# miemie2013/Pytorch-PPYOLO

Measured on AMD Instinct MI355X. Metric: images/sec PPYOLO R50-vd 608x608 bs=8, higher is better.
Workload: dtype f32; 1 GPU; PPYOLO ResNet50-vd (DCNv2, CoordConv, SPP) 608x608, 8 images per GPU, device-resident input -> padded detections; global_batch=8, parallelism=single GPU, hip_graph=True, tile_table=tuned_gfx950_f16x2.json

## Files before the change

pytorch-ppyolo_amd/ppyolo_hip/csrc/conv_shared.h:

```cpp
#pragma once
#include "common.h"

#ifndef PPY_X3_BBLOCK
#define PPY_X3_BBLOCK 1
#endif

struct ConvArgs {
    const float *x, *w, *scale, *shift, *res, *posb;
    const unsigned short *w3;
    const unsigned short *wf16;
    const float *scale_f16;
    const float *posb_f16;
    const float *amax_in;
    const float *amax_in2 = nullptr;
    float *amax_out;
    float *y, *part;
    int x_ld, res_ld, y_ld;
    int N, H, W, C, Ho, Wo, K, R, S, stride, pad, act, ups;
    int M, Kred, cchunks, chunks_total, chunks_per_split;
    int nstages;
    int panel_n = 0;
    unsigned long long *trace;
    float *bn_part = nullptr;
    int *bn_slices_host = nullptr;
    int bn_capacity = 0;
    int bn_nostore = 0;
    const float *bn_mean = nullptr, *bn_invstd = nullptr, *bn_gamma = nullptr, *bn_beta = nullptr;
    float *yscale = nullptr;
    float ysplit_mul = 0.f, ysplit_add = 0.f;
    const float *xscale = nullptr;
};

static __device__ __forceinline__ float split_scale_of(float bound) {
    const int e = (int)((__float_as_uint(bound) >> 23) & 0xffu);
    int f = 267 - e;
    f = f < 103 ? 103 : (f > 167 ? 167 : f);
    return __uint_as_float((unsigned)f << 23);
}
static __device__ __forceinline__ float pow2_above(float mx) {
    const unsigned e = (__float_as_uint(mx) >> 23) & 0xffu;
    return __uint_as_float((e >= 253u ? 254u : e + 1u) << 23);
}
static __device__ __forceinline__ float pow2_inverse(float s) {
    return __uint_as_float((254u - ((__float_as_uint(s) >> 23) & 0xffu)) << 23);
}

#if defined(__HIPCC__)
static __device__ __forceinline__ float conv_amax_in(const ConvArgs &p, int n) {
    float mx = amax_read(p.amax_in, n);
    if (p.amax_in2) mx = fmaxf(mx, amax_read(p.amax_in2, n));
    return mx;
}
#endif

struct Geometry {
    int Ho, Wo, M, Kred, chunks;
};

static inline ppy_conv_cfg_info ppy_cfg_info(int family, int local, int operands, int bm, int bn, int stages, int splitk_mode,
                                             bool reads_presplit, bool writes_presplit, bool bn_stats, int stats_twin = -1) {
    return ppy_conv_cfg_info{family, local, operands, bm, bn, stages, splitk_mode, reads_presplit, writes_presplit, bn_stats, stats_twin};
}

int ppy_x3_num_configs();
int ppy_x3_f16_base();
int ppy_x3_config_info(int local_cfg, ppy_conv_cfg_info *out);
int ppy_x3_dispatch(const ConvArgs &p, int local_cfg, int splits, hipStream_t stream);
static inline int ppy_panel_n(const ConvArgs &p, int BM, int BN, int splits) {
    static const int mode = getenv("PPY_TILE_PANEL") ? atoi(getenv("PPY_TILE_PANEL")) : 1;
    if (mode == 0 || splits > 1) return 0;
    const int tiles_m = (p.M + BM - 1) / BM, tiles_n = (p.K + BN - 1) / BN;
    if (tiles_m * tiles_n < 16) return 0;
    const double A = (double)p.N * p.H * p.W * p.C * 4.0, W = (double)p.K * p.Kred * 4.0;
    int best = 1;
    double best_cost = A + 8.0 * W;
    for (int gn = 2; gn <= 8; gn *= 2) {
        if (gn > tiles_n || 8 / gn > tiles_m) continue;
        if (mode > 1 && gn != mode) continue;
        const double cost = gn * A + (8.0 / gn) * W;
        if (cost < 0.9 * best_cost || (mode > 1 && gn == mode)) { best = gn; best_cost = cost; }
    }
    return best == 1 ? 0 : (tiles_n + best - 1) / best;
}
#if defined(__HIPCC__)
__device__ __forceinline__ void ppy_tile_of(const ConvArgs &p, int tiles_n, int &tile_m, int &tile_n) {
    const int nb = (int)gridDim.x, q = nb >> 3, r = nb & 7;
    const int xcd = (int)blockIdx.x & 7, idx = (int)blockIdx.x >> 3;
    const int tile_id = xcd * q + min(xcd, r) + idx;
    const int pn = p.panel_n;
    if (pn <= 0 || pn >= tiles_n) {
        tile_m = tile_id / tiles_n;
        tile_n = tile_id - tile_m * tiles_n;
        return;
    }
    const int tiles_m = nb / tiles_n, per_panel = tiles_m * pn;
    const int panel = tile_id / per_panel, within = tile_id - panel * per_panel;
    const int pw = min(pn, tiles_n - panel * pn);
    tile_m = within / pw;
    tile_n = panel * pn + (within - tile_m * pw);
}
#endif

int ppy_stream_num_configs();
int ppy_stream_config_info(int local_cfg, ppy_conv_cfg_info *out);
int ppy_stream_dispatch(const ConvArgs &p, int local_cfg, float *pool, int pool_ld, hipStream_t stream);
int ppy_patch_num_configs();
int ppy_patch_config_info(int local_cfg, ppy_conv_cfg_info *out);
int ppy_patch_dispatch(const ConvArgs &p, int local_cfg, hipStream_t stream);
int ppy_patch_maxpool_dispatch(const ConvArgs &p, int Hp, int Wp, hipStream_t stream);
int ppy_ws_num_configs();
int ppy_ws_config_info(int local_cfg, ppy_conv_cfg_info *out);
int ppy_ws_dispatch(const ConvArgs &p, int local_cfg, int splits, hipStream_t stream);
int ppy_small_num_configs();
int ppy_small_config_info(int local_cfg, ppy_conv_cfg_info *out);
int ppy_small_dispatch(const ConvArgs &p, int local_cfg, int splits, hipStream_t stream);

namespace {

constexpr int BK = 32;
constexpr int LDS_LD = 36;

typedef __attribute__((ext_vector_type(8))) __bf16 bf16x8;
typedef __attribute__((ext_vector_type(2))) __bf16 bf16x2;
typedef __attribute__((ext_vector_type(2))) float floatx2;
typedef __attribute__((ext_vector_type(4))) unsigned uintx4;
typedef __attribute__((ext_vector_type(8))) _Float16 f16x8;
typedef __attribute__((ext_vector_type(2))) _Float16 f16x2;

__device__ __forceinline__ unsigned cvt_pk_f16(float a, float b) {
    const floatx2 v = {a, b};
    return __builtin_bit_cast(unsigned, __builtin_convertvector(v, f16x2));
}
__device__ __forceinline__ float f16_lo(unsigned p) { return (float)__builtin_bit_cast(_Float16, (unsigned short)(p & 0xffffu)); }
__device__ __forceinline__ float f16_hi(unsigned p) { return (float)__builtin_bit_cast(_Float16, (unsigned short)(p >> 16)); }

__device__ __forceinline__ unsigned cvt_pk_bf16(float a, float b) {
    const floatx2 v = {a, b};
    return __builtin_bit_cast(unsigned, __builtin_convertvector(v, bf16x2));
}

__device__ __forceinline__ float epilogue_store(const ConvArgs &p, int m, int col, float v,
                                                float sc, float sh) {
    const int hw = p.Ho * p.Wo;
    if (p.posb) v += p.posb[(long long)(m % hw) * p.K + col];
    v = fmaf(v, sc, sh);
    if (p.res) v += p.res[(long long)m * p.res_ld + col];
    v = ppy_apply_act(v, p.act);
    if (!p.ups) {
        p.y[(long long)m * p.y_ld + col] = v;
    } else {
        const int n = m / hw, rem = m - n * hw;
        const int ho = rem / p.Wo, wo = rem - ho * p.Wo;
        const long long W2 = 2LL * p.Wo;
        float *o = p.y + (((long long)n * 2 * p.Ho + 2 * ho) * W2 + 2 * wo) * p.y_ld + col;
        o[0] = v;
        o[p.y_ld] = v;
        o[W2 * p.y_ld] = v;
        o[(W2 + 1) * p.y_ld] = v;
    }
    return v;
}

template <int TM, int TN, int WM, int WN, bool SPLIT, bool VEC>
__device__ __forceinline__ void tile_epilogue(const ConvArgs &p, floatx16 (&acc)[TM][TN], float *smem, int m0,
                                              int n0, int wm, int wn, int lane, int wave, int split,
                                              const float (*rowscale)[4] = nullptr, const float (*rowsplit)[4] = nullptr,
                                              bool split_out = false) {
    const int hw = p.Ho * p.Wo;
    if constexpr (VEC) {
        float *sE = smem + wave * (32 * LDS_LD);
        const int erow = lane >> 3, ec4 = (lane & 7) * 4;
        const int mw0 = min(m0 + wm * WM, p.M - 1), mw1 = min(m0 + wm * WM + WM - 1, p.M - 1);
        const int n_lo = mw0 / hw, n_hi = mw1 / hw;
        const int bnd = (n_lo + 1) * hw;
        float amx = 0.0f, amx_hi = 0.0f;
        floatx4 rv[TM][TN][4];
        if (!SPLIT && p.res) {
#pragma unroll
            for (int j = 0; j < TN; ++j)
#pragma unroll
                for (int i = 0; i < TM; ++i)
#pragma unroll
                    for (int t = 0; t < 4; ++t) {
                        const int col = n0 + wn * WN + j * 32 + ec4;
                        const int m = m0 + wm * WM + i * 32 + erow + 8 * t;
                        rv[i][j][t] = floatx4{0.f, 0.f, 0.f, 0.f};
                        if (col < p.K && m < p.M)
                            rv[i][j][t] = *reinterpret_cast<const floatx4 *>(p.res + (long long)m * p.res_ld + col);
                    }
        } else if (!SPLIT && p.posb) {
#pragma unroll
            for (int j = 0; j < TN; ++j)
#pragma unroll
                for (int i = 0; i < TM; ++i)
#pragma unroll
                    for (int t = 0; t < 4; ++t) {
                        const int col = n0 + wn * WN + j * 32 + ec4;
                        const int m = m0 + wm * WM + i * 32 + erow + 8 * t;
                        rv[i][j][t] = floatx4{0.f, 0.f, 0.f, 0.f};
                        if (col < p.K && m < p.M)
                            rv[i][j][t] = *reinterpret_cast<const floatx4 *>(p.posb + (long long)(m % hw) * p.K + col);
                    }
        }
        constexpr bool HOIST_SC = TM * TN < 4;
        floatx4 scv[HOIST_SC ? TN : 1], shv[HOIST_SC ? TN : 1];
        if constexpr (HOIST_SC) {
#pragma unroll
            for (int j = 0; j < TN; ++j) {
                const int col = n0 + wn * WN + j * 32 + ec4;
                scv[j] = floatx4{1.f, 1.f, 1.f, 1.f};
                shv[j] = floatx4{0.f, 0.f, 0.f, 0.f};
                if (!SPLIT && col < p.K) {
                    scv[j] = *reinterpret_cast<const floatx4 *>(p.scale + col);
                    shv[j] = *reinterpret_cast<const floatx4 *>(p.shift + col);
                }
            }
            if (!SPLIT) {
#pragma unroll
                for (int j = 0; j < TN; ++j) asm volatile("" : "+v"(scv[j]), "+v"(shv[j]));
            }
        }
        if (!SPLIT && (p.res || p.posb)) {
#pragma unroll
            for (int j = 0; j < TN; ++j)
#pragma unroll
                for (int i = 0; i < TM; ++i)
#pragma unroll
                    for (int t = 0; t < 4; ++t) asm volatile("" : "+v"(rv[i][j][t]));
        }
#pragma unroll
        for (int j = 0; j < TN; ++j) {
            const int col = n0 + wn * WN + j * 32 + ec4;
            const bool colok = col < p.K;
            floatx4 sc = {1.f, 1.f, 1.f, 1.f}, sh = {0.f, 0.f, 0.f, 0.f};
            if constexpr (HOIST_SC) {
                sc = scv[j];
                sh = shv[j];
            } else if (!SPLIT) {
                if (colok) {
                    sc = *reinterpret_cast<const floatx4 *>(p.scale + col);
                    sh = *reinterpret_cast<const floatx4 *>(p.shift + col);
                }
                asm volatile("" : "+v"(sc), "+v"(sh));
            }
#pragma unroll
            for (int i = 0; i < TM; ++i) {
                const int mbase = m0 + wm * WM + i * 32 + erow;
#pragma unroll
                for (int e = 0; e < 16; ++e) {
                    const int row = (e & 3) + 8 * (e >> 2) + 4 * (lane >> 5);
                    sE[row * LDS_LD + (lane & 31)] = acc[i][j][e];
                }
                __builtin_amdgcn_wave_barrier();
#pragma unroll
                for (int t = 0; t < 4; ++t) {
                    const int m = mbase + 8 * t;
                    floatx4 v = *reinterpret_cast<const floatx4 *>(sE + (erow + 8 * t) * LDS_LD + ec4);
                    if (rowscale) {
#pragma unroll
                        for (int u = 0; u < 4; ++u) v[u] *= rowscale[i][t];
                    }
                    if (colok && m < p.M) {
                        if (SPLIT) {
                            *reinterpret_cast<floatx4 *>(p.part + ((long long)split * p.M + m) * p.K + col) = v;
                        } else {
                            if (p.posb) {
                                floatx4 pb = rv[i][j][t];
                                if (p.res) {
                                    pb = *reinterpret_cast<const floatx4 *>(p.posb + (long long)(m % hw) * p.K + col);
                                    asm volatile("" : "+v"(pb));
                                }
#pragma unroll
                                for (int u = 0; u < 4; ++u) v[u] += pb[u];
                            }
#pragma unroll
                            for (int u = 0; u < 4; ++u) {
                                float o = fmaf(v[u], sc[u], sh[u]);
                                if (p.res) o += rv[i][j][t][u];
                                v[u] = ppy_apply_act(o, p.act);
                            }
                            {
                                const float rmx = fmaxf(fmaxf(fabsf(v[0]), fabsf(v[1])), fmaxf(fabsf(v[2]), fabsf(v[3])));
                                amx = fmaxf(amx, m < bnd ? rmx : 0.0f);
                                amx_hi = fmaxf(amx_hi, m < bnd ? 0.0f : rmx);
                            }
                            if (rowsplit != nullptr && split_out) {
                                typedef __attribute__((ext_vector_type(2))) unsigned uintx2_;
                                const float s = rowsplit[i][t];
                                const unsigned h0 = cvt_pk_f16(v[0] * s, v[1] * s), h1 = cvt_pk_f16(v[2] * s, v[3] * s);
                                const unsigned l0 = cvt_pk_f16(fmaf(v[0], s, -f16_lo(h0)), fmaf(v[1], s, -f16_hi(h0)));
                                const unsigned l1 = cvt_pk_f16(fmaf(v[2], s, -f16_lo(h1)), fmaf(v[3], s, -f16_hi(h1)));
                                char *o = reinterpret_cast<char *>(p.y + (long long)m * p.y_ld) + (col >> 5) * 128 + (col & 31) * 2;
                                *reinterpret_cast<uintx2_ *>(o) = uintx2_{h0, h1};
                                *reinterpret_cast<uintx2_ *>(o + 64) = uintx2_{l0, l1};
                            } else if (!p.ups) {
                                *reinterpret_cast<floatx4 *>(p.y + (long long)m * p.y_ld + col) = v;
                            } else {
                                const int n = m / hw, rem = m - n * hw;
                                const int ho = rem / p.Wo, wo = rem - ho * p.Wo;
                                const long long W2 = 2LL * p.Wo;
                                float *o = p.y + (((long long)n * 2 * p.Ho + 2 * ho) * W2 + 2 * wo) * p.y_ld + col;
                                *reinterpret_cast<floatx4 *>(o) = v;
                                *reinterpret_cast<floatx4 *>(o + p.y_ld) = v;
                                *reinterpret_cast<floatx4 *>(o + W2 * p.y_ld) = v;
                                *reinterpret_cast<floatx4 *>(o + (W2 + 1) * p.y_ld) = v;
                            }
                        }
                    }
                }
                __builtin_amdgcn_wave_barrier();
            }
        }
        if (!SPLIT && p.amax_out) amax_track2(amx, amx_hi, n_lo, n_hi, p.amax_out, blockIdx.x * 8 + wave);
        return;
    }
    float amx = 0.0f, amx_hi = 0.0f;
    const int mw0 = min(m0 + wm * WM, p.M - 1), mw1 = min(m0 + wm * WM + WM - 1, p.M - 1);
    const int n_lo = mw0 / hw, n_hi = mw1 / hw;
    const int bnd = (n_lo + 1) * hw;
#pragma unroll
    for (int j = 0; j < TN; ++j) {
        const int col = n0 + wn * WN + j * 32 + (lane & 31);
        const bool colok = col < p.K;
        float sc = 1.f, sh = 0.f;
        if (!SPLIT && colok) {
            sc = p.scale[col];
            sh = p.shift[col];
        }
#pragma unroll
        for (int i = 0; i < TM; ++i) {
#pragma unroll
            for (int e = 0; e < 16; ++e) {
                const int row = (e & 3) + 8 * (e >> 2) + 4 * (lane >> 5);
                const int m = m0 + wm * WM + i * 32 + row;
                if (colok && m < p.M) {
                    if (SPLIT)
                        p.part[((long long)split * p.M + m) * p.K + col] = acc[i][j][e];
                    else
                    {
                        const float a = fabsf(epilogue_store(p, m, col, acc[i][j][e], sc, sh));
                        amx = fmaxf(amx, m < bnd ? a : 0.0f);
                        amx_hi = fmaxf(amx_hi, m < bnd ? 0.0f : a);
                    }
                }
            }
        }
    }
    if (!SPLIT && p.amax_out) amax_track2(amx, amx_hi, n_lo, n_hi, p.amax_out, blockIdx.x * 8 + wave);
}

template <int TM, int TN, int WM, int WN>
__device__ __forceinline__ void tile_bn_stats(const ConvArgs &p, const floatx16 (&acc)[TM][TN], const float (&inv_sa)[TM], int m0, int n0,
                                              int wm, int wn, int lane, int slice) {
    const int row0 = m0 + wm * WM;
    const int nvalid = min(max(p.M - row0, 0), WM);
    float inv[TM][16];
#pragma unroll
    for (int i = 0; i < TM; ++i)
#pragma unroll
        for (int e = 0; e < 16; ++e) inv[i][e] = __shfl(inv_sa[i], (e & 3) + 8 * (e >> 2) + 4 * (lane >> 5));
#pragma unroll
    for (int j = 0; j < TN; ++j) {
        const int col = n0 + wn * WN + j * 32 + (lane & 31);
        const bool colok = col < p.K;
        const float sc = colok ? p.scale[col] : 1.f, sh = colok ? p.shift[col] : 0.f;
        float sum = 0.f;
#pragma unroll
        for (int i = 0; i < TM; ++i)
#pragma unroll
            for (int e = 0; e < 16; ++e) {
                const int r = i * 32 + (e & 3) + 8 * (e >> 2) + 4 * (lane >> 5);
                const float v = fmaf(acc[i][j][e] * inv[i][e], sc, sh);
                sum += r < nvalid ? v : 0.f;
            }
        sum += __shfl_xor(sum, 32);
        const float mean = nvalid > 0 ? sum / (float)nvalid : 0.f;
        float m2 = 0.f;
#pragma unroll
        for (int i = 0; i < TM; ++i)
#pragma unroll
            for (int e = 0; e < 16; ++e) {
                const int r = i * 32 + (e & 3) + 8 * (e >> 2) + 4 * (lane >> 5);
                const float d = fmaf(acc[i][j][e] * inv[i][e], sc, sh) - mean;
                m2 += r < nvalid ? d * d : 0.f;
            }
        m2 += __shfl_xor(m2, 32);
        if (colok && lane < 32) {
            float *o = p.bn_part + ((long long)slice * p.K + col) * 3;
            o[0] = (float)nvalid;
            o[1] = mean;
            o[2] = m2;
        }
    }
}

__device__ __forceinline__ void split8(const floatx4 lo, const floatx4 hi, bf16x8 (&out)[3]) {
    uintx4 p0, p1, p2;
#pragma unroll
    for (int q = 0; q < 4; ++q) {
        const float a = q < 2 ? lo[2 * q] : hi[2 * q - 4], b = q < 2 ? lo[2 * q + 1] : hi[2 * q - 3];
        const unsigned P0 = cvt_pk_bf16(a, b);
        const float ra = a - __uint_as_float(P0 << 16), rb = b - __uint_as_float(P0 & 0xffff0000u);
        const unsigned P1 = cvt_pk_bf16(ra, rb);
        const float sa = ra - __uint_as_float(P1 << 16), sb = rb - __uint_as_float(P1 & 0xffff0000u);
        p0[q] = P0;
        p1[q] = P1;
        p2[q] = cvt_pk_bf16(sa, sb);
    }
    out[0] = __builtin_bit_cast(bf16x8, p0);
    out[1] = __builtin_bit_cast(bf16x8, p1);
    out[2] = __builtin_bit_cast(bf16x8, p2);
}

template <int N>
__device__ __forceinline__ void wait_vmcnt() {
    asm volatile("s_waitcnt vmcnt(%0)" ::"n"(N) : "memory");
}

template <bool VEC>
__global__ void __launch_bounds__(256) splitk_reduce_kernel(const ConvArgs p, int splits) {
    constexpr int W = VEC ? 4 : 1;
    const long long total = (long long)p.M * p.K;
    const long long i = ((long long)blockIdx.x * 256 + threadIdx.x) * W;
    float amx = 0.0f;
    if (i < total) {
    const int m = (int)(i / p.K), col = (int)(i - (long long)m * p.K);
    if constexpr (VEC) {
        floatx4 v = *reinterpret_cast<const floatx4 *>(p.part + i);
        for (int z0 = 1; z0 < splits; z0 += 8) {
            floatx4 o[8];
#pragma unroll
            for (int q = 0; q < 8; ++q)
                if (z0 + q < splits) o[q] = *reinterpret_cast<const floatx4 *>(p.part + (long long)(z0 + q) * total + i);
#pragma unroll
            for (int q = 0; q < 8; ++q)
                if (z0 + q < splits) {
#pragma unroll
                    for (int u = 0; u < 4; ++u) v[u] += o[q][u];
                }
        }
        const floatx4 sc = *reinterpret_cast<const floatx4 *>(p.scale + col);
        const floatx4 sh = *reinterpret_cast<const floatx4 *>(p.shift + col);
        if (p.posb) {
            const floatx4 pb = *reinterpret_cast<const floatx4 *>(p.posb + (long long)(m % (p.Ho * p.Wo)) * p.K + col);
#pragma unroll
            for (int u = 0; u < 4; ++u) v[u] += pb[u];
        }
        floatx4 r = {0.f, 0.f, 0.f, 0.f};
        if (p.res) r = *reinterpret_cast<const floatx4 *>(p.res + (long long)m * p.res_ld + col);
#pragma unroll
        for (int u = 0; u < 4; ++u) {
            v[u] = ppy_apply_act(fmaf(v[u], sc[u], sh[u]) + (p.res ? r[u] : 0.f), p.act);
            amx = fmaxf(amx, fabsf(v[u]));
        }
        if (!p.ups) {
            *reinterpret_cast<floatx4 *>(p.y + (long long)m * p.y_ld + col) = v;
        } else {
            const int hw = p.Ho * p.Wo, n = m / hw, rem = m - n * hw;
            const int ho = rem / p.Wo, wo = rem - ho * p.Wo;
            const long long W2 = 2LL * p.Wo;
            float *o = p.y + (((long long)n * 2 * p.Ho + 2 * ho) * W2 + 2 * wo) * p.y_ld + col;
            *reinterpret_cast<floatx4 *>(o) = v;
            *reinterpret_cast<floatx4 *>(o + p.y_ld) = v;
            *reinterpret_cast<floatx4 *>(o + W2 * p.y_ld) = v;
            *reinterpret_cast<floatx4 *>(o + (W2 + 1) * p.y_ld) = v;
        }
    } else {
        float v = p.part[i];
        for (int z0 = 1; z0 < splits; z0 += 8) {
            float o[8];
#pragma unroll
            for (int q = 0; q < 8; ++q)
                if (z0 + q < splits) o[q] = p.part[(long long)(z0 + q) * total + i];
#pragma unroll
            for (int q = 0; q < 8; ++q)
                if (z0 + q < splits) v += o[q];
        }
        amx = fabsf(epilogue_store(p, m, col, v, p.scale[col], p.shift[col]));
    }
    }
    if (p.amax_out) {
        const long long ic = i < total ? i : total - 1;
        amax_track(amx, (int)(ic / p.K) / (p.Ho * p.Wo), p.amax_out, blockIdx.x * 4 + (threadIdx.x >> 6));
    }
}

inline void launch_splitk_reduce(const ConvArgs &p, int splits, bool vec, hipStream_t stream) {
    const long long total = (long long)p.M * p.K;
    const long long threads = vec ? total / 4 : total;
    const unsigned grid = (unsigned)((threads + 255) / 256);
    if (vec)
        hipLaunchKernelGGL(splitk_reduce_kernel<true>, dim3(grid), dim3(256), 0, stream, p, splits);
    else
        hipLaunchKernelGGL(splitk_reduce_kernel<false>, dim3(grid), dim3(256), 0, stream, p, splits);
}

bool vec_epilogue_ok(const ConvArgs &p) {
    auto al = [](const void *q) { return ((uintptr_t)q & 15) == 0; };
    if (p.K % 4 != 0 || p.y_ld % 4 != 0 || !al(p.y) || !al(p.scale) || !al(p.shift)) return false;
    if (p.res && (p.res_ld % 4 != 0 || !al(p.res))) return false;
    if (p.posb && !al(p.posb)) return false;
    if (p.part && !al(p.part)) return false;
    return true;
}


bool conv_geometry(int N, int H, int W, int C, int K, int R, int S, int stride, int pad, Geometry *g) {
    if (N <= 0 || H <= 0 || W <= 0 || C <= 0 || K <= 0 || R <= 0 || S <= 0 || stride <= 0 || pad < 0)
        return false;
    if (C % BK != 0) return false;
    const int Ho = (H + 2 * pad - R) / stride + 1, Wo = (W + 2 * pad - S) / stride + 1;
    if (Ho <= 0 || Wo <= 0) return false;
    const long long M = (long long)N * Ho * Wo;
    if (M > 0x7fffffffLL / 4) return false;
    g->Ho = Ho;
    g->Wo = Wo;
    g->M = (int)M;
    g->Kred = R * S * C;
    g->chunks = R * S * (C / BK);
    return true;
}

}
```

pytorch-ppyolo_amd/ppyolo_hip/csrc/conv_ws.hip:

```cpp
#include "conv_shared.h"

#include <type_traits>

namespace {

template <int BM, int BN, int NS, bool SPLIT, bool VEC, bool BNS = false, bool PRE = false, bool GP = false, bool KP = false, int CPS = 1>
__global__ void __launch_bounds__((BM == 256 || KP) ? 768 : 512) conv_igemm_ws_kernel(const ConvArgs p) {
#if defined(__HIP_DEVICE_COMPILE__)
    static_assert(!KP || (BM <= 128 && !PRE && !BNS), "k-parity consumers: 64- / 128-row tiles, plain / pre-split input, no BatchNorm statistics");
    static_assert(CPS == 1 || (CPS == 2 && KP), "two chunks per stage: the k-parity tiles");
    constexpr int CM = BM == 256 ? 4 : 2, NC = CM * 2 * (KP ? 2 : 1);
    constexpr int WM = BM / CM, WN = BN / 2, TM = WM / 32, TN = WN / 32;
    constexpr int NP = 2, B_ROWS = NP * BN, NWP = 4;
    static_assert(BM % (8 * NWP) == 0 && B_ROWS % (16 * NWP) == 0, "whole DMA instructions per producer wave");
    constexpr int A_PASS = BM / (8 * NWP), B_PASS = B_ROWS / (16 * NWP), G = CPS * (A_PASS + B_PASS);
    constexpr int A_BYTES = BM * 128, AP_BYTES = PRE ? 2 * BM * 64 : 0, B_BYTES = B_ROWS * 64;
    constexpr int SUB = A_BYTES + AP_BYTES + B_BYTES, STAGE = CPS * SUB;
    static_assert((NS - 1) * G <= 63, "6-bit vmcnt");
    static_assert(!GP || (!PRE && !SPLIT && VEC && !BNS), "pre-split input: plain consumers, one split, vector epilogue");
    typedef __attribute__((address_space(3))) void *lds_ptr;
    extern __shared__ __attribute__((aligned(16))) char smem_ws[];
    char *smem = smem_ws;

    const int tid = threadIdx.x, lane = tid & 63;
    const int wave = __builtin_amdgcn_readfirstlane(tid >> 6);
    const int tiles_n = (p.K + BN - 1) / BN;
    int tile_m, tile_n;
    ppy_tile_of(p, tiles_n, tile_m, tile_n);
    const int m0 = tile_m * BM, n0 = tile_n * BN;
    const int split = blockIdx.y;
    const int kc_begin = split * p.chunks_per_split;
    const int kc_end = min(kc_begin + p.chunks_per_split, p.chunks_total);
    const int nchunks = kc_end - kc_begin;
    const int nsuper = (nchunks + CPS - 1) / CPS;
    const int hw = p.Ho * p.Wo;

    if (wave >= NC) {
        const int pw = wave - NC;
        const unsigned OOB = 0xFFFFFFF0u;
        const long long bias = (long long)(p.pad * p.W + p.pad) * p.x_ld * 4;
        unsigned a_off[A_PASS], a_ok[A_PASS], b_off[B_PASS];
        {
            const int drow = lane >> 3, dslot = lane & 7;
            const int step_rows = 8 * NWP;
            const int step_ho = step_rows / p.Wo, step_wo = step_rows - step_ho * p.Wo;
            int m_first = min(m0 + pw * 8 + drow, p.M - 1);
            int n = m_first / hw, rem = m_first - n * hw;
            int ho = rem / p.Wo, wo = rem - ho * p.Wo;
#pragma unroll
            for (int j = 0; j < A_PASS; ++j) {
                const int row = (j * NWP + pw) * 8 + drow;
                const int scol = dslot ^ ((row >> 1) & 7);
                const int mr = m0 + row;
                const int hi0 = ho * p.stride - p.pad, wi0 = wo * p.stride - p.pad;
                a_off[j] = (unsigned)((((long long)n * p.H + hi0) * p.W + wi0) * p.x_ld * 4 + bias + scol * 16);
                unsigned colmask = 0, okb = 0;
                for (int s2 = 0; s2 < p.S; ++s2)
                    if ((unsigned)(wi0 + s2) < (unsigned)p.W) colmask |= 1u << s2;
                for (int r = 0; r < p.R; ++r)
                    if ((unsigned)(hi0 + r) < (unsigned)p.H) okb |= colmask << (r * p.S);
                a_ok[j] = mr < p.M ? okb : 0u;
                wo += step_wo;
                ho += step_ho;
                if (wo >= p.Wo) { wo -= p.Wo; ++ho; }
                while (ho >= p.Ho) { ho -= p.Ho; ++n; }
            }
        }
        {
            const int drow = lane >> 2, dslot = lane & 3;
            const long long plane_bytes = (long long)p.K * p.Kred * 2;
#pragma unroll
            for (int j = 0; j < B_PASS; ++j) {
                const int rb = (j * NWP + pw) * 16 + drow;
                const int plane = rb / BN, nrow = rb - plane * BN;
                const int scol = dslot ^ ((rb >> 2) & 3);
                const int k = min(n0 + nrow, p.K - 1);
                b_off[j] = (unsigned)(plane * plane_bytes + (long long)k * 64 + scol * 16);
            }
        }
        const int RS = p.R * p.S;
        int l_cc = kc_begin / RS, l_tap = kc_begin - l_cc * RS;
        int l_r = l_tap / p.S, l_s = l_tap - l_r * p.S;
        const char *xb = reinterpret_cast<const char *>(p.x) - bias;
        const char *wb = reinterpret_cast<const char *>(p.wf16);
        auto issue_sub = [&](int lds_base, bool have) {
            const long long a_uni = ((long long)(l_r * p.W + l_s) * p.x_ld + l_cc * 32) * 4;
            const long long b_uni = ((long long)l_tap * (p.C / 32) + l_cc) * p.K * 64;
            const __amdgpu_buffer_rsrc_t ra = __builtin_amdgcn_make_buffer_rsrc((void *)(xb + (have ? a_uni : 0)), 0, 0xFFFFFF00u, 0x00020000);
            const __amdgpu_buffer_rsrc_t rb = __builtin_amdgcn_make_buffer_rsrc((void *)(wb + (have ? b_uni : 0)), 0, 0xFFFFFF00u, 0x00020000);
            const unsigned tapbit = have ? (1u << l_tap) : 0u;
            const unsigned lds = (unsigned)(lds_base + pw * 1024);
#pragma unroll
            for (int d = 0; d < A_PASS; ++d) {
                const unsigned off = (a_ok[d] & tapbit) ? a_off[d] : OOB;
                __builtin_amdgcn_raw_ptr_buffer_load_lds(ra, (lds_ptr)(smem + lds + d * NWP * 1024), 16, off, 0, 0, 0);
            }
#pragma unroll
            for (int j = 0; j < B_PASS; ++j) {
                const unsigned off = have ? b_off[j] : OOB;
                __builtin_amdgcn_raw_ptr_buffer_load_lds(rb, (lds_ptr)(smem + lds + A_BYTES + AP_BYTES + j * NWP * 1024), 16, off, 0, 0, 0);
            }
            ++l_tap;
            ++l_s;
            if (l_s == p.S) { l_s = 0; ++l_r; }
            if (l_tap == RS) { l_tap = 0; l_r = 0; l_s = 0; ++l_cc; }
        };
        auto issue = [&](int stage, int sup) {
#pragma unroll
            for (int u = 0; u < CPS; ++u) issue_sub(stage * STAGE + u * SUB, sup * CPS + u < nchunks);
        };
        float sa_p[A_PASS];
        if constexpr (PRE) {
#pragma unroll
            for (int j = 0; j < A_PASS; ++j) {
                const int mrow = min(m0 + (j * NWP + pw) * 8 + (lane >> 3), p.M - 1);
                const float mx = conv_amax_in(p, mrow / hw);
                const int e = (int)((__float_as_uint(mx) >> 23) & 0xffu);
                int f = 267 - e;
                f = f < 103 ? 103 : (f > 167 ? 167 : f);
                sa_p[j] = __uint_as_float((unsigned)f << 23);
            }
        }
        auto split_stage = [&](int stage) {
            if constexpr (PRE) {
                typedef __attribute__((ext_vector_type(2))) unsigned uintx2;
                char *sb = smem + stage * STAGE;
#pragma unroll
                for (int d = 0; d < A_PASS; ++d) {
                    const int row = (d * NWP + pw) * 8 + (lane >> 3);
                    const int g4 = (lane & 7) ^ ((row >> 1) & 7);
                    const floatx4 v = *reinterpret_cast<const floatx4 *>(sb + pw * 1024 + d * NWP * 1024 + lane * 16);
                    const float sc_r = sa_p[d];
                    const unsigned h0 = cvt_pk_f16(v[0] * sc_r, v[1] * sc_r), h1 = cvt_pk_f16(v[2] * sc_r, v[3] * sc_r);
                    const unsigned l0 = cvt_pk_f16(fmaf(v[0], sc_r, -f16_lo(h0)), fmaf(v[1], sc_r, -f16_hi(h0)));
                    const unsigned l1 = cvt_pk_f16(fmaf(v[2], sc_r, -f16_lo(h1)), fmaf(v[3], sc_r, -f16_hi(h1)));
                    const int o = row * 64 + (((g4 >> 1) ^ ((row >> 2) & 3)) << 4) + (g4 & 1) * 8;
                    *reinterpret_cast<uintx2 *>(sb + A_BYTES + o) = uintx2{h0, h1};
                    *reinterpret_cast<uintx2 *>(sb + A_BYTES + BM * 64 + o) = uintx2{l0, l1};
                }
                asm volatile("s_waitcnt lgkmcnt(0)" ::: "memory");
            }
        };
        if (nchunks > 0) {
#pragma unroll
            for (int sidx = 0; sidx < NS; ++sidx) issue(sidx, sidx);
            wait_vmcnt<(NS - 1) * G>();
            split_stage(0);
            __builtin_amdgcn_s_barrier();
            int st = 0;
            for (int k = 0; k < nsuper; ++k) {
                wait_vmcnt<(NS - 2) * G>();
                split_stage(st + 1 == NS ? 0 : st + 1);
                __builtin_amdgcn_s_barrier();
                issue(st, k + NS);
                st = st + 1 == NS ? 0 : st + 1;
            }
            asm volatile("s_waitcnt vmcnt(0)" ::: "memory");
            __builtin_amdgcn_s_barrier();
        }
        return;
    }

    const int grp = KP ? wave >> 2 : 0;
    const int wq = KP ? wave & 3 : wave;
    const int wm = wq >> 1, wn = wq & 1;
    floatx16 acc[TM][TN];
#pragma unroll
    for (int i = 0; i < TM; ++i)
#pragma unroll
        for (int j = 0; j < TN; ++j)
#pragma unroll
            for (int e = 0; e < 16; ++e) acc[i][j][e] = 0.f;
    const int frow = lane & 31, fkh = lane >> 5;
    const int a_sw = (frow >> 1) & 7, b_sw = (frow >> 2) & 3;
    int a_foff[2][2], b_foff[2];
#pragma unroll
    for (int s = 0; s < 2; ++s) {
        if constexpr (GP) {
            a_foff[s][0] = frow * 128 + (((2 * s + fkh) ^ a_sw) << 4);
            a_foff[s][1] = frow * 128 + (((4 + 2 * s + fkh) ^ a_sw) << 4);
        } else {
            a_foff[s][0] = frow * 128 + (((4 * s + 2 * fkh) ^ a_sw) << 4);
            a_foff[s][1] = frow * 128 + (((4 * s + 2 * fkh + 1) ^ a_sw) << 4);
        }
        b_foff[s] = frow * 64 + (((2 * s + fkh) ^ b_sw) << 4);
    }
    int ap_foff[2];
#pragma unroll
    for (int s = 0; s < 2; ++s) ap_foff[s] = frow * 64 + (((2 * s + fkh) ^ b_sw) << 4);
    float sa[TM], inv_sa[TM], xmax_up[TM];
#pragma unroll
    for (int i = 0; i < TM; ++i) {
        xmax_up[i] = 1.0f;
        const int mrow = min(m0 + wm * WM + i * 32 + (lane & 31), p.M - 1);
        if constexpr (GP) {
            sa[i] = p.xscale[mrow / hw];
            inv_sa[i] = pow2_inverse(sa[i]);
            if (p.yscale) xmax_up[i] = pow2_above(conv_amax_in(p, mrow / hw));
            continue;
        }
        const float mx = conv_amax_in(p, mrow / hw);
        const int e = (int)((__float_as_uint(mx) >> 23) & 0xffu);
        int f = 267 - e;
        f = f < 103 ? 103 : (f > 167 ? 167 : f);
        sa[i] = __uint_as_float((unsigned)f << 23);
        inv_sa[i] = __uint_as_float((unsigned)(254 - f) << 23);
        xmax_up[i] = 16384.0f * inv_sa[i];
    }

    struct Frag {
        uintx4 a[TM][NP];
        uintx4 b[NP][TN];
    };
    constexpr int NM = 3 * TM * TN;
    constexpr int NRA = 2 * TM, NRB = NP * TN, NR = NRA + NRB;
    constexpr int NSL = (PRE || GP) ? 0 : 3 * 4 * TM;
    constexpr int RPS = (NR + NM - 1) / NM;
    constexpr int LEAD0 = (NRA + RPS - 1) / RPS + 1;
    constexpr int LEAD = LEAD0 < NM ? LEAD0 : NM - 1;
    constexpr int PER = (NSL + (NM - LEAD) - 1) / (NM - LEAD);
    auto step = [&](const Frag &cur, Frag &nxt, int stage, const int ao0, const int ao1, const int bo, const int apo) {
        constexpr int ta[3] = {1, 0, 0}, tb[3] = {0, 1, 0};
        const char *a_ptr = PRE ? smem + stage * STAGE + A_BYTES + wm * WM * 64 : smem + stage * STAGE + wm * WM * 128;
        const char *b_ptr = smem + stage * STAGE + A_BYTES + AP_BYTES + wn * WN * 64;
        floatx4 raw[TM][2];
        float ra[TM][4], rb[TM][4];
#pragma unroll
        for (int m = 0; m < NM; ++m) {
            {
                const int t = m / (TM * TN), i = (m / TN) % TM, j = m % TN;
                acc[i][j] = __builtin_amdgcn_mfma_f32_32x32x16_f16(__builtin_bit_cast(f16x8, cur.a[i][ta[t]]),
                                                                  __builtin_bit_cast(f16x8, cur.b[tb[t]][j]), acc[i][j], 0, 0, 0);
            }
#pragma unroll
            for (int u = 0; u < RPS; ++u) {
                const int r = m * RPS + u;
                if (r >= NR) {
                } else if (r < NRA) {
                    if constexpr (PRE)
                        nxt.a[r >> 1][r & 1] = *reinterpret_cast<const uintx4 *>(a_ptr + (r & 1) * BM * 64 + (r >> 1) * 32 * 64 + apo);
                    else if constexpr (GP)
                        nxt.a[r >> 1][r & 1] = *reinterpret_cast<const uintx4 *>(a_ptr + (r >> 1) * 32 * 128 + ((r & 1) ? ao1 : ao0));
                    else
                        raw[r >> 1][r & 1] = *reinterpret_cast<const floatx4 *>(a_ptr + (r >> 1) * 32 * 128 + ((r & 1) ? ao1 : ao0));
                } else {
                    const int pl = (r - NRA) / TN, j = (r - NRA) % TN;
                    nxt.b[pl][j] = *reinterpret_cast<const uintx4 *>(b_ptr + (pl * BN + j * 32) * 64 + bo);
                }
            }
            if (m >= LEAD) {
#pragma unroll
                for (int u = 0; u < PER; ++u) {
                    const int sl = (m - LEAD) * PER + u;
                    if (sl < NSL) {
                        const int st = sl / (4 * TM), pr = sl % (4 * TM), i = pr / 4, q = pr % 4;
                        const float xa = raw[i][q >> 1][(q & 1) * 2], xb = raw[i][q >> 1][(q & 1) * 2 + 1];
                        if (st == 0) {
                            nxt.a[i][0][q] = cvt_pk_f16(xa * sa[i], xb * sa[i]);
                        } else if (st == 1) {
                            const unsigned P = nxt.a[i][0][q];
                            ra[i][q] = fmaf(xa, sa[i], -f16_lo(P));
                            rb[i][q] = fmaf(xb, sa[i], -f16_hi(P));
                        } else {
                            nxt.a[i][1][q] = cvt_pk_f16(ra[i][q], rb[i][q]);
                        }
                    }
                }
            }
            __builtin_amdgcn_sched_barrier(0);
        }
#pragma unroll
        for (int i = 0; i < TM; ++i)
#pragma unroll
            for (int pl = 0; pl < NP; ++pl) asm volatile("" : "+v"(nxt.a[i][pl]));
    };
    const int o_a0 = (KP && grp) ? a_foff[1][0] : a_foff[0][0], o_a1 = (KP && grp) ? a_foff[1][1] : a_foff[0][1];
    const int o_b = (KP && grp) ? b_foff[1] : b_foff[0], o_ap = (KP && grp) ? ap_foff[1] : ap_foff[0];

    if (nchunks > 0) {
        Frag f0, f1;
        __builtin_amdgcn_s_barrier();
        {
            const char *a_ptr = smem + wm * WM * 128;
            const char *b_ptr = smem + A_BYTES + AP_BYTES + wn * WN * 64;
#pragma unroll
            for (int i = 0; i < TM; ++i) {
                if constexpr (PRE) {
#pragma unroll
                    for (int pl = 0; pl < 2; ++pl)
                        f0.a[i][pl] = *reinterpret_cast<const uintx4 *>(smem + A_BYTES + pl * BM * 64 + (wm * WM + i * 32) * 64 + o_ap);
                    continue;
                }
                if constexpr (GP) {
                    f0.a[i][0] = *reinterpret_cast<const uintx4 *>(a_ptr + i * 32 * 128 + o_a0);
                    f0.a[i][1] = *reinterpret_cast<const uintx4 *>(a_ptr + i * 32 * 128 + o_a1);
                    continue;
                }
                const floatx4 lo = *reinterpret_cast<const floatx4 *>(a_ptr + i * 32 * 128 + o_a0);
                const floatx4 hi = *reinterpret_cast<const floatx4 *>(a_ptr + i * 32 * 128 + o_a1);
#pragma unroll
                for (int q = 0; q < 4; ++q) {
                    const float xa = q < 2 ? lo[2 * q] : hi[2 * q - 4], xb = q < 2 ? lo[2 * q + 1] : hi[2 * q - 3];
                    const unsigned P0 = cvt_pk_f16(xa * sa[i], xb * sa[i]);
                    f0.a[i][0][q] = P0;
                    f0.a[i][1][q] = cvt_pk_f16(fmaf(xa, sa[i], -f16_lo(P0)), fmaf(xb, sa[i], -f16_hi(P0)));
                }
            }
#pragma unroll
            for (int pl = 0; pl < NP; ++pl)
#pragma unroll
                for (int j = 0; j < TN; ++j)
                    f0.b[pl][j] = *reinterpret_cast<const uintx4 *>(b_ptr + (pl * BN + j * 32) * 64 + o_b);
        }
        int st = 0;
        if constexpr (KP && CPS == 2) {
            for (int k = 0; k < nsuper; ++k) {
                step(f0, f1, st, o_a0 + SUB, o_a1 + SUB, o_b + SUB, o_ap);
                asm volatile("s_waitcnt lgkmcnt(0)" ::: "memory");
                __builtin_amdgcn_s_barrier();
                st = st + 1 == NS ? 0 : st + 1;
                step(f1, f0, st, o_a0, o_a1, o_b, o_ap);
            }
        } else if constexpr (KP) {
            auto sync = [&]() {
                asm volatile("s_waitcnt lgkmcnt(0)" ::: "memory");
                __builtin_amdgcn_s_barrier();
                st = st + 1 == NS ? 0 : st + 1;
            };
            int k = 0;
            for (; k + 2 <= nchunks; k += 2) {
                sync();
                step(f0, f1, st, o_a0, o_a1, o_b, o_ap);
                sync();
                step(f1, f0, st, o_a0, o_a1, o_b, o_ap);
            }
            if (k < nchunks) {
                sync();
                step(f0, f1, st, o_a0, o_a1, o_b, o_ap);
            }
        } else {
            for (int k = 0; k < nchunks; ++k) {
                step(f0, f1, st, a_foff[1][0], a_foff[1][1], b_foff[1], ap_foff[1]);
                asm volatile("s_waitcnt lgkmcnt(0)" ::: "memory");
                __builtin_amdgcn_s_barrier();
                st = st + 1 == NS ? 0 : st + 1;
                step(f1, f0, st, a_foff[0][0], a_foff[0][1], b_foff[0], ap_foff[0]);
            }
        }
        asm volatile("s_waitcnt lgkmcnt(0)" ::: "memory");
        __builtin_amdgcn_s_barrier();
    }
    if constexpr (BNS) tile_bn_stats<TM, TN, WM, WN>(p, acc, inv_sa, m0, n0, wm, wn, lane, tile_m * CM + wm);
    float rowscale[TM][4], rowsplit[TM][4];
#pragma unroll
    for (int i = 0; i < TM; ++i)
#pragma unroll
        for (int t = 0; t < 4; ++t) rowsplit[i][t] = 0.f;
    bool split_out = false;
    if constexpr (VEC && !SPLIT) {
        split_out = p.yscale != nullptr;
        if (split_out) {
#pragma unroll
            for (int i = 0; i < TM; ++i) {
                const float ys = split_scale_of(fmaf(p.ysplit_mul, xmax_up[i], p.ysplit_add));
                const int mr = m0 + wm * WM + i * 32 + (lane & 31);
                if (n0 == 0 && wn == 0 && lane < 32 && mr < p.M) p.yscale[mr / hw] = ys;
#pragma unroll
                for (int t = 0; t < 4; ++t) rowsplit[i][t] = __shfl(ys, (lane >> 3) + 8 * t);
            }
        }
    }
    if constexpr (VEC) {
#pragma unroll
        for (int i = 0; i < TM; ++i)
#pragma unroll
            for (int t = 0; t < 4; ++t) rowscale[i][t] = __shfl(inv_sa[i], (lane >> 3) + 8 * t);
    } else {
#pragma unroll
        for (int i = 0; i < TM; ++i)
#pragma unroll
            for (int e = 0; e < 16; ++e) {
                const float inv = __shfl(inv_sa[i], (e & 3) + 8 * (e >> 2) + 4 * (lane >> 5));
#pragma unroll
                for (int j = 0; j < TN; ++j) acc[i][j][e] *= inv;
            }
    }
    if constexpr (KP) {
        static_assert(!KP || TN == 2, "one column half per group");
        constexpr int XCH_OFF = 40960, XCH_WAVE = TM * 16 * 64;
        float *xch = reinterpret_cast<float *>(smem + XCH_OFF);
#pragma unroll
        for (int i = 0; i < TM; ++i)
#pragma unroll
            for (int e = 0; e < 16; ++e) xch[wave * XCH_WAVE + (i * 16 + e) * 64 + lane] = grp ? acc[i][0][e] : acc[i][1][e];
        asm volatile("s_waitcnt lgkmcnt(0)" ::: "memory");
        __builtin_amdgcn_s_barrier();
        floatx16 half[TM][1];
#pragma unroll
        for (int i = 0; i < TM; ++i)
#pragma unroll
            for (int e = 0; e < 16; ++e) {
                const float theirs = xch[(wave ^ 4) * XCH_WAVE + (i * 16 + e) * 64 + lane];
                half[i][0][e] = grp ? theirs + acc[i][1][e] : acc[i][0][e] + theirs;
            }
        tile_epilogue<TM, 1, WM, 32, SPLIT, VEC>(p, half, reinterpret_cast<float *>(smem), m0, n0, wm, 2 * wn + grp, lane, wave, split,
                                                 VEC ? rowscale : nullptr, (VEC && !SPLIT) ? rowsplit : nullptr, split_out);
    } else {
        tile_epilogue<TM, TN, WM, WN, SPLIT, VEC>(p, acc, reinterpret_cast<float *>(smem), m0, n0, wm, wn, lane, wave, split,
                                                  VEC ? rowscale : nullptr, (VEC && !SPLIT) ? rowsplit : nullptr, split_out);
    }
#endif
}

template <int BM, int BN, int NS, bool PRE, bool SPLIT, bool VEC, bool BNS = false, bool GP = false, bool KP = false, int CPS = 1>
int launch_ws_one(const ConvArgs &p, int splits, size_t lds, int tiles, hipStream_t stream) {
    if constexpr (!SPLIT && !BNS && !GP && !KP) {
        if (p.bn_part) return launch_ws_one<BM, BN, NS, PRE, SPLIT, VEC, true>(p, splits, lds, tiles, stream);
    }
    if constexpr (!SPLIT && VEC && !BNS && !PRE && !GP) {
        if (p.xscale) return launch_ws_one<BM, BN, NS, PRE, SPLIT, VEC, false, true, KP, CPS>(p, splits, lds, tiles, stream);
    }
    auto k = conv_igemm_ws_kernel<BM, BN, NS, SPLIT, VEC, BNS, PRE, GP, KP, CPS>;
    static PpyLdsAttr attr;
    if (ppy_lds_attr(attr, reinterpret_cast<const void *>(k), 160 * 1024) != PPY_OK) return PPY_ERR_LAUNCH;
    hipLaunchKernelGGL(k, dim3(tiles, splits), dim3((BM == 256 || KP) ? 768 : 512), lds, stream, p);
    return PPY_OK;
}

template <int BM, int BN, int NS, bool PRE = false, bool KP = false, int CPS = 1>
int launch_ws(ConvArgs p, int splits, hipStream_t stream) {
    const long long xbytes = (long long)p.N * p.H * p.W * p.x_ld * 4 + (long long)(p.pad * p.W + p.pad) * p.x_ld * 4;
    const long long wbytes = (long long)p.K * p.Kred * 2 * 2;
    if (xbytes >= 0xFFFFF000LL || wbytes >= 0xFFFFF000LL || p.R * p.S > 32) return PPY_ERR_UNSUPPORTED;
    constexpr int STAGE_BYTES = CPS * (BM * 128 * (PRE ? 2 : 1) + 2 * BN * 64);
    static_assert(NS * STAGE_BYTES <= 160 * 1024, "LDS");
    size_t lds = (size_t)NS * STAGE_BYTES;
    const size_t epi = KP ? (size_t)40960 + 8 * (BM / 64) * 16 * 64 * sizeof(float)
                          : (size_t)(BM == 256 ? 8 : 4) * 32 * LDS_LD * sizeof(float);
    if (lds < epi) lds = epi;
    if (KP && p.bn_part) return PPY_ERR_UNSUPPORTED;
    p.nstages = NS;
    p.chunks_total = p.R * p.S * (p.C / 32);
    p.chunks_per_split = ceil_div(p.chunks_total, splits);
    splits = ceil_div(p.chunks_total, p.chunks_per_split);
    const int tiles = ceil_div(p.M, BM) * ceil_div(p.K, BN);
    p.panel_n = ppy_panel_n(p, BM, BN, splits);
    const bool vec = vec_epilogue_ok(p);
    if (p.bn_part) {
        if (splits > 1 || p.res || p.posb || p.ups || p.act != PPY_ACT_NONE) return PPY_ERR_UNSUPPORTED;
        if (ceil_div(p.M, BM) * (BM == 256 ? 4 : 2) > p.bn_capacity) return PPY_ERR_WORKSPACE;
        if (p.bn_slices_host) *p.bn_slices_host = ceil_div(p.M, BM) * (BM == 256 ? 4 : 2);
    }
    if ((p.xscale || p.yscale) && (splits > 1 || !vec || p.bn_part)) return PPY_ERR_BAD_ARG;
    if (p.yscale && p.ups) return PPY_ERR_BAD_ARG;
    if (p.xscale && PRE) return PPY_ERR_BAD_ARG;
    if (p.yscale && (p.K % 32 != 0 || p.y_ld % 32 != 0)) return PPY_ERR_BAD_ARG;
    int rc;
    if (splits > 1) {
        rc = vec ? launch_ws_one<BM, BN, NS, PRE, true, true, false, false, KP, CPS>(p, splits, lds, tiles, stream)
                 : launch_ws_one<BM, BN, NS, PRE, true, false, false, false, KP, CPS>(p, splits, lds, tiles, stream);
        if (rc != PPY_OK) return rc;
        launch_splitk_reduce(p, splits, vec, stream);
    } else {
        rc = vec ? launch_ws_one<BM, BN, NS, PRE, false, true, false, false, KP, CPS>(p, splits, lds, tiles, stream)
                 : launch_ws_one<BM, BN, NS, PRE, false, false, false, false, KP, CPS>(p, splits, lds, tiles, stream);
        if (rc != PPY_OK) return rc;
    }
    return ppy_launch_status();
}

}

struct WsCfg {
    int bm, bn, ns;
    bool pre, kp;
    int cps, twin;
};
constexpr WsCfg kWs[] = {
    {128, 128, 3, false, false, 1, -1},
    {128, 128, 4, false, false, 1, -1},
    {64, 128, 4, false, false, 1, -1},
    {64, 128, 6, false, false, 1, -1},
    {128, 128, 3, true, false, 1, -1},
    {64, 128, 4, true, false, 1, -1},
    {128, 64, 4, true, false, 1, -1},
    {256, 128, 2, false, false, 1, -1},
    {256, 128, 3, false, false, 1, -1},
    {128, 128, 3, false, true, 1, 0},
    {128, 128, 4, false, true, 1, 1},
    {64, 128, 4, false, true, 1, 2},
    {64, 128, 6, false, true, 1, 3},
    {128, 128, 2, false, true, 2, 1},
    {64, 128, 2, false, true, 2, 2},
    {64, 128, 3, false, true, 2, 3},
};
#define WS_CASE(i) case i: return launch_ws<kWs[i].bm, kWs[i].bn, kWs[i].ns, kWs[i].pre, kWs[i].kp, kWs[i].cps>(q, s, st)
int ppy_ws_num_configs() { return sizeof(kWs) / sizeof(kWs[0]); }

int ppy_ws_config_info(int c, ppy_conv_cfg_info *out) {
    if (c < 0 || c >= ppy_ws_num_configs()) return PPY_ERR_BAD_ARG;
    const WsCfg &t = kWs[c];
    *out = ppy_cfg_info(t.pre ? PPY_CFG_WS_PRE : (t.kp ? PPY_CFG_WS_KPARITY : PPY_CFG_WS), c, PPY_CFG_OPERANDS_F16X2, t.bm, t.bn, t.ns,
                        PPY_CFG_SPLITK_WORKSPACE, !t.pre, true, !t.kp, t.twin);
    return PPY_OK;
}

int ppy_ws_dispatch(const ConvArgs &p, int c, int s, hipStream_t st) {
    if (!p.wf16 || ((uintptr_t)p.wf16 & 15) != 0 || !p.scale_f16 || !p.amax_in || (p.posb && !p.posb_f16)) return PPY_ERR_BAD_ARG;
    ConvArgs q = p;
    q.scale = p.scale_f16;
    q.posb = p.posb ? p.posb_f16 : nullptr;
    switch (c) {
        WS_CASE(0);
        WS_CASE(1);
        WS_CASE(2);
        WS_CASE(3);
        WS_CASE(4);
        WS_CASE(5);
        WS_CASE(6);
        WS_CASE(7);
        WS_CASE(8);
        WS_CASE(9);
        WS_CASE(10);
        WS_CASE(11);
        WS_CASE(12);
        WS_CASE(13);
        WS_CASE(14);
        WS_CASE(15);
        static_assert(sizeof(kWs) / sizeof(kWs[0]) == 16, "one case per descriptor");
    }
    return PPY_ERR_BAD_ARG;
}
```

Before: 2474 images/s.

## Prefetch residual tile into freed pipeline stages via DMA producer waves

Producer waves in the warp-specialized implicit-GEMM conv now use the final NS pipeline slots, once the K-loop has no more chunks to load, to DMA the residual (or optionally position-bias) tile into LDS with buffer_load_lds. Consumers read it from LDS into registers before the epilogue, so residual global loads leave the critical tail. The k-parity path also keeps its own half-accumulator in registers instead of re-reading acc. This adds register pressure, an extra barrier and LDS-offset bookkeeping. It is on by default for residual convs, with env overrides.

```diff
diff --git a/pytorch-ppyolo_amd/ppyolo_hip/csrc/conv_shared.h b/pytorch-ppyolo_amd/ppyolo_hip/csrc/conv_shared.h
--- a/pytorch-ppyolo_amd/ppyolo_hip/csrc/conv_shared.h
+++ b/pytorch-ppyolo_amd/ppyolo_hip/csrc/conv_shared.h
@@ -29,6 +29,7 @@
     float *yscale = nullptr;
     float ysplit_mul = 0.f, ysplit_add = 0.f;
     const float *xscale = nullptr;
+    int res_pref = 0;
 };
 
 static __device__ __forceinline__ float split_scale_of(float bound) {
@@ -161,11 +162,11 @@
     return v;
 }
 
-template <int TM, int TN, int WM, int WN, bool SPLIT, bool VEC>
+template <int TM, int TN, int WM, int WN, bool SPLIT, bool VEC, bool RVPRE = false>
 __device__ __forceinline__ void tile_epilogue(const ConvArgs &p, floatx16 (&acc)[TM][TN], float *smem, int m0,
                                               int n0, int wm, int wn, int lane, int wave, int split,
                                               const float (*rowscale)[4] = nullptr, const float (*rowsplit)[4] = nullptr,
-                                              bool split_out = false) {
+                                              bool split_out = false, const floatx4 (*rv_pre)[TN][4] = nullptr, bool rv_have = false) {
     const int hw = p.Ho * p.Wo;
     if constexpr (VEC) {
         float *sE = smem + wave * (32 * LDS_LD);
@@ -175,7 +176,20 @@
         const int bnd = (n_lo + 1) * hw;
         float amx = 0.0f, amx_hi = 0.0f;
         floatx4 rv[TM][TN][4];
-        if (!SPLIT && p.res) {
+        bool rv_given = false;
+        if constexpr (RVPRE && !SPLIT) {
+            if (rv_have) {
+                rv_given = true;
+#pragma unroll
+                for (int j = 0; j < TN; ++j)
+#pragma unroll
+                    for (int i = 0; i < TM; ++i)
+#pragma unroll
+                        for (int t = 0; t < 4; ++t) rv[i][j][t] = rv_pre[i][j][t];
+            }
+        }
+        if (rv_given) {
+        } else if (!SPLIT && p.res) {
 #pragma unroll
             for (int j = 0; j < TN; ++j)
 #pragma unroll
diff --git a/pytorch-ppyolo_amd/ppyolo_hip/csrc/conv_ws.hip b/pytorch-ppyolo_amd/ppyolo_hip/csrc/conv_ws.hip
--- a/pytorch-ppyolo_amd/ppyolo_hip/csrc/conv_ws.hip
+++ b/pytorch-ppyolo_amd/ppyolo_hip/csrc/conv_ws.hip
@@ -18,6 +18,9 @@
     constexpr int SUB = A_BYTES + AP_BYTES + B_BYTES, STAGE = CPS * SUB;
     static_assert((NS - 1) * G <= 63, "6-bit vmcnt");
     static_assert(!GP || (!PRE && !SPLIT && VEC && !BNS), "pre-split input: plain consumers, one split, vector epilogue");
+    constexpr int G1 = A_PASS + B_PASS, SUB_PIECES = NWP * G1;
+    constexpr int RV_PIECES = BM * BN / 256, RV_BN = BN / 32;
+    constexpr bool RVP = VEC && !SPLIT && !BNS && NS * CPS * SUB_PIECES >= RV_PIECES;
     typedef __attribute__((address_space(3))) void *lds_ptr;
     extern __shared__ __attribute__((aligned(16))) char smem_ws[];
     char *smem = smem_ws;
@@ -34,6 +37,12 @@
     const int nchunks = kc_end - kc_begin;
     const int nsuper = (nchunks + CPS - 1) / CPS;
     const int hw = p.Ho * p.Wo;
+    const int rv_s0 = nsuper % NS;
+    auto rv_lds_off = [&](int id) {
+        const int q = id / SUB_PIECES, e = id - q * SUB_PIECES, j = q / CPS, u = q - j * CPS;
+        const int stage = rv_s0 + j >= NS ? rv_s0 + j - NS : rv_s0 + j;
+        return stage * STAGE + u * SUB + e * 1024 + (e >= NWP * A_PASS ? AP_BYTES : 0);
+    };
 
     if (wave >= NC) {
         const int pw = wave - NC;
@@ -109,6 +118,36 @@
 #pragma unroll
             for (int u = 0; u < CPS; ++u) issue_sub(stage * STAGE + u * SUB, sup * CPS + u < nchunks);
         };
+        const bool rv_on = RVP && p.res_pref;
+        const int rv_ld4 = (p.res ? p.res_ld : p.K) * 4;
+        const int rv_rows = p.M - m0 - (lane >> 3), rv_cols = p.K - n0 - (lane & 7) * 4;
+        const unsigned rv_lane = (unsigned)((lane >> 3) * rv_ld4 + (lane & 7) * 16);
+        const int rv_rem = rv_on && !p.res ? (m0 + (lane >> 3)) % hw : 0;
+        const bool rv_wrap1 = hw >= BM + 8;
+        const char *rv_base = reinterpret_cast<const char *>(p.res ? p.res + (long long)m0 * p.res_ld + n0 : p.posb + n0);
+        const __amdgpu_buffer_rsrc_t rv_rsrc = __builtin_amdgcn_make_buffer_rsrc((void *)rv_base, 0, 0xFFFFFF00u, 0x00020000);
+        const bool rv_res = p.res != nullptr;
+        auto issue_rv = [&](int stage, int j) {
+#pragma unroll
+            for (int u = 0; u < CPS; ++u)
+#pragma unroll
+                for (int d = 0; d < G1; ++d) {
+                    const int id = ((j * CPS + u) * G1 + d) * NWP + pw;
+                    const int rb = id / RV_BN, cb = id - rb * RV_BN;
+                    unsigned off;
+                    if (rv_res) {
+                        off = rv_lane + (unsigned)(rb * 8 * rv_ld4 + cb * 128);
+                    } else {
+                        int r = rv_rem + rb * 8;
+                        if (rv_wrap1) r -= r >= hw ? hw : 0;
+                        else r %= hw;
+                        off = (unsigned)(r * rv_ld4 + cb * 128 + (lane & 7) * 16);
+                    }
+                    const bool ok = id < RV_PIECES && rb * 8 < rv_rows && cb * 32 < rv_cols;
+                    __builtin_amdgcn_raw_ptr_buffer_load_lds(rv_rsrc, (lds_ptr)(smem + stage * STAGE + u * SUB + pw * 1024 + (d < A_PASS ? d : d - A_PASS) * NWP * 1024 +
+                                                                                (d < A_PASS ? 0 : A_BYTES + AP_BYTES)), 16, ok ? off : OOB, 0, 0, 0);
+                }
+        };
         float sa_p[A_PASS];
         if constexpr (PRE) {
 #pragma unroll
@@ -143,16 +182,27 @@
         };
         if (nchunks > 0) {
 #pragma unroll
-            for (int sidx = 0; sidx < NS; ++sidx) issue(sidx, sidx);
+            for (int sidx = 0; sidx < NS; ++sidx) {
+                if (rv_on && sidx >= nsuper) issue_rv(sidx, sidx - nsuper);
+                else issue(sidx, sidx);
+            }
             wait_vmcnt<(NS - 1) * G>();
             split_stage(0);
             __builtin_amdgcn_s_barrier();
-            int st = 0;
-            for (int k = 0; k < nsuper; ++k) {
+            int st = 0, k = 0;
+            for (; k < nsuper - NS; ++k) {
                 wait_vmcnt<(NS - 2) * G>();
                 split_stage(st + 1 == NS ? 0 : st + 1);
                 __builtin_amdgcn_s_barrier();
                 issue(st, k + NS);
+                st = st + 1 == NS ? 0 : st + 1;
+            }
+            for (; k < nsuper; ++k) {
+                wait_vmcnt<(NS - 2) * G>();
+                split_stage(st + 1 == NS ? 0 : st + 1);
+                __builtin_amdgcn_s_barrier();
+                if (rv_on) issue_rv(st, k + NS - nsuper);
+                else issue(st, k + NS);
                 st = st + 1 == NS ? 0 : st + 1;
             }
             asm volatile("s_waitcnt vmcnt(0)" ::: "memory");
@@ -350,6 +400,25 @@
         asm volatile("s_waitcnt lgkmcnt(0)" ::: "memory");
         __builtin_amdgcn_s_barrier();
     }
+    constexpr int RTN = KP ? 1 : TN;
+    floatx4 rvp[TM][RTN][4];
+    bool rv_have = false;
+    if constexpr (RVP) {
+        rv_have = p.res_pref != 0 && nchunks > 0;
+        if (rv_have) {
+#pragma unroll
+            for (int j = 0; j < RTN; ++j)
+#pragma unroll
+                for (int i = 0; i < TM; ++i)
+#pragma unroll
+                    for (int t = 0; t < 4; ++t) {
+                        const int id = (wm * (WM / 8) + i * 4 + t) * RV_BN + (KP ? 2 * wn + grp : wn * TN + j);
+                        rvp[i][j][t] = *reinterpret_cast<const floatx4 *>(smem + rv_lds_off(id) + lane * 16);
+                    }
+            asm volatile("s_waitcnt lgkmcnt(0)" ::: "memory");
+            __builtin_amdgcn_s_barrier();
+        }
+    }
     if constexpr (BNS) tile_bn_stats<TM, TN, WM, WN>(p, acc, inv_sa, m0, n0, wm, wn, lane, tile_m * CM + wm);
     float rowscale[TM][4], rowsplit[TM][4];
 #pragma unroll
@@ -389,25 +458,30 @@
         static_assert(!KP || TN == 2, "one column half per group");
         constexpr int XCH_OFF = 40960, XCH_WAVE = TM * 16 * 64;
         float *xch = reinterpret_cast<float *>(smem + XCH_OFF);
+        floatx16 half[TM][1];
 #pragma unroll
         for (int i = 0; i < TM; ++i)
 #pragma unroll
-            for (int e = 0; e < 16; ++e) xch[wave * XCH_WAVE + (i * 16 + e) * 64 + lane] = grp ? acc[i][0][e] : acc[i][1][e];
+            for (int e = 0; e < 16; ++e) {
+                xch[wave * XCH_WAVE + (i * 16 + e) * 64 + lane] = grp ? acc[i][0][e] : acc[i][1][e];
+                half[i][0][e] = grp ? acc[i][1][e] : acc[i][0][e];
+            }
         asm volatile("s_waitcnt lgkmcnt(0)" ::: "memory");
+#pragma unroll
+        for (int i = 0; i < TM; ++i) asm volatile("" : "+v"(half[i][0]));
         __builtin_amdgcn_s_barrier();
-        floatx16 half[TM][1];
 #pragma unroll
         for (int i = 0; i < TM; ++i)
 #pragma unroll
             for (int e = 0; e < 16; ++e) {
                 const float theirs = xch[(wave ^ 4) * XCH_WAVE + (i * 16 + e) * 64 + lane];
-                half[i][0][e] = grp ? theirs + acc[i][1][e] : acc[i][0][e] + theirs;
-            }
-        tile_epilogue<TM, 1, WM, 32, SPLIT, VEC>(p, half, reinterpret_cast<float *>(smem), m0, n0, wm, 2 * wn + grp, lane, wave, split,
-                                                 VEC ? rowscale : nullptr, (VEC && !SPLIT) ? rowsplit : nullptr, split_out);
+                half[i][0][e] = grp ? theirs + half[i][0][e] : half[i][0][e] + theirs;
+            }
+        tile_epilogue<TM, 1, WM, 32, SPLIT, VEC, RVP>(p, half, reinterpret_cast<float *>(smem), m0, n0, wm, 2 * wn + grp, lane, wave, split,
+                                                      VEC ? rowscale : nullptr, (VEC && !SPLIT) ? rowsplit : nullptr, split_out, rvp, rv_have);
     } else {
-        tile_epilogue<TM, TN, WM, WN, SPLIT, VEC>(p, acc, reinterpret_cast<float *>(smem), m0, n0, wm, wn, lane, wave, split,
-                                                  VEC ? rowscale : nullptr, (VEC && !SPLIT) ? rowsplit : nullptr, split_out);
+        tile_epilogue<TM, TN, WM, WN, SPLIT, VEC, RVP>(p, acc, reinterpret_cast<float *>(smem), m0, n0, wm, wn, lane, wave, split,
+                                                       VEC ? rowscale : nullptr, (VEC && !SPLIT) ? rowsplit : nullptr, split_out, rvp, rv_have);
     }
 #endif
 }
@@ -455,6 +529,12 @@
     if (p.yscale && p.ups) return PPY_ERR_BAD_ARG;
     if (p.xscale && PRE) return PPY_ERR_BAD_ARG;
     if (p.yscale && (p.K % 32 != 0 || p.y_ld % 32 != 0)) return PPY_ERR_BAD_ARG;
+    p.res_pref = 0;
+    if (splits == 1 && vec && (p.res || p.posb)) {
+        const char *sw = getenv("PPY_WS_RES_OLD"), *pb = getenv("PPY_WS_POSB_PREF");
+        const long long rvbytes = p.res ? (long long)p.M * p.res_ld * 4 : (long long)p.Ho * p.Wo * p.K * 4;
+        if (!(sw && sw[0] == '1') && (p.res || (pb && pb[0] == '1')) && rvbytes < 0xFFFFF000LL) p.res_pref = 1;
+    }
     int rc;
     if (splits > 1) {
         rc = vec ? launch_ws_one<BM, BN, NS, PRE, true, true, false, false, KP, CPS>(p, splits, lds, tiles, stream)
```

Measured after the change: 2471 images/s. Within noise of the previous version (-0.1%).
